# atenpas/gpd

Hardware: NVIDIA H100
Metric: grasp candidates/sec end-to-end (15ch) (higher is better)
Workload: dtype f64 geometry / f32 LeNet

## Files before the change

### gpd_b200/csrc/geometry.cu

```cuda
#include <cfloat>
#include <climits>
#include <cstdlib>
#include <vector>
#include <cub/cub.cuh>

#include "common.cuh"
#include "grid.cuh"

namespace {

constexpr int NT_HANDS = 256;
#ifndef GPDB_NT_IMG
#define GPDB_NT_IMG 512
#endif
constexpr int NT_IMG = GPDB_NT_IMG;
constexpr int LRF_WARPS = 4;
constexpr int LRF_CAP_GLOBAL = 16384;
constexpr int LRF_CAP = 1024;
constexpr int BOX_CAP = 2048;
constexpr int MAXPIX = 64 * 64;

__device__ __forceinline__ void to_frame(const double *F, double v0, double v1, double v2, double &o0, double &o1,
                                         double &o2) {
  o0 = (F[0] * v0 + F[1] * v1) + F[2] * v2;
// ... 1059 lines not shown
}
__device__ __forceinline__ void unit_axis(double v, double lo, double extent, double inv_extent, int S, double &u, int &cell) {
  u = (v - lo) * inv_extent;
  double q = u * (double)S;
  double fq = floor(q);
  const double fr = q - fq;
  if (fr < 1e-9 || fr > 1.0 - 1e-9) {
    u = (v - lo) / extent;
    double cellsize = 1.0 / (double)S;
    fq = floor(u / cellsize);
  }
  cell = min((int)fq, S - 1);
}
__device__ __forceinline__ unsigned unit_q32(double u) {
  return __double2uint_rz(u * 4294967296.0);
}

constexpr int RCP_N = (NT_IMG / 32) * 4;
__device__ __forceinline__ double cell_mean(unsigned long long acc, const double *rcp) {
  const unsigned c = (unsigned)(acc >> 48);
  const double sum = (double)(acc & 0xffffffffffffull);
  return c < (unsigned)RCP_N ? sum * rcp[c] : sum / ((double)c * 4294967296.0);
}

__device__ __forceinline__ bool fully_covered(const unsigned *occf, int S);
template <int NT, int NV>
__device__ __forceinline__ void block_max(float (&v)[NV], float (*red)[8], const unsigned *occf = nullptr, int S = 0,
                                          bool *covered = nullptr) {
#pragma unroll
  for (int o = 16; o; o >>= 1)
#pragma unroll
    for (int i = 0; i < NV; i++) v[i] = fmaxf(v[i], __shfl_xor_sync(0xffffffffu, v[i], o));
  __syncthreads();
  if ((threadIdx.x & 31) == 0)
#pragma unroll
    for (int i = 0; i < NV; i++) red[threadIdx.x >> 5][i] = v[i];
  if (occf && threadIdx.x < 32) {
    const bool c = fully_covered(occf, S);
    if (threadIdx.x == 0) red[0][7] = c ? 1.0f : 0.0f;
  }
  __syncthreads();
#pragma unroll
  for (int i = 0; i < NV; i++) v[i] = red[0][i];
  for (int w = 1; w < NT / 32; w++)
#pragma unroll
    for (int i = 0; i < NV; i++) v[i] = fmaxf(v[i], red[w][i]);
// ... 231 lines not shown
      unit_axis(x, h.bottom, P.vol_d, inv_d, S, u0, c0);
      unit_axis(y, h.center - P.vol_w / 2.0, P.vol_w, inv_w, S, u1, c1);
      unit_axis(z, -P.vol_h, 2.0 * P.vol_h, inv_h, S, u2, c2);
      bq[k] = unit_q32(u0);
      bq[BC + k] = unit_q32(u1);
      bq[2 * BC + k] = unit_q32(u2);
      bcell[k] = (unsigned)c0 | ((unsigned)c1 << 8) | ((unsigned)c2 << 16);
      const double *nn = cl.nrm + 3 * (size_t)(unsigned)(bkeys[k] & 0xffffffffull);
      double n0, n1, n2;
      to_frame(h.frame, nn[0], nn[1], nn[2], n0, n1, n2);
      bnrm[k] = (float)fabs(n0);
      bnrm[BC + k] = (float)fabs(n1);
      bnrm[2 * BC + k] = (float)fabs(n2);
      if (!unit_normal(nn)) nonunit = true;
    }
    const bool exact_fold = __syncthreads_or(nonunit) != 0;

    for (int pj = 0; pj < nproj; pj++) {
      const int a0 = (pj == 0) ? 0 : 2, a1 = (pj == 2) ? 0 : 1, a2 = (pj == 0) ? 2 : (pj == 1 ? 0 : 1);
      for (int k = tid; k < bn; k += NT_IMG) {
        const unsigned cc = bcell[k];
        const int row = S - 1 - (int)((cc >> (8 * a0)) & 255), col = (cc >> (8 * a1)) & 255;
        const int pix = row * S + col;
        atomicMax(tileA + pix, bkeys[k]);
        atomicAdd(tileB + pix, (1ull << 48) + (unsigned long long)bq[a2 * BC + k]);
        atomicOr(&sm.occf[pix >> 5], 1u << (pix & 31));
      }
      __syncthreads();
      auto cell_values = [&](int k, int &row, int &col, float &n0, float &n1, float &n2, float &dv) -> bool {
        const unsigned cc = bcell[k];
        row = S - 1 - (int)((cc >> (8 * a0)) & 255);
        col = (cc >> (8 * a1)) & 255;
        const int pix = row * S + col;
        if (tileA[pix] != bkeys[k]) return false;
        n0 = bnrm[k];
        n1 = bnrm[BC + k];
        n2 = bnrm[2 * BC + k];
        if (exact_fold) {
          float v0 = 0.0f, v1 = 0.0f, v2 = 0.0f;
          unsigned long long cur = 0ull;
          bool first = true;
          for (;;) {
            unsigned long long nxt = ~0ull;
            int jn = k;
            for (int j = 0; j < bn; j++) {
              const unsigned cj = bcell[j];
              const unsigned long long kj = bkeys[j];
              if ((S - 1 - (int)((cj >> (8 * a0)) & 255)) * S + (int)((cj >> (8 * a1)) & 255) == pix && (first || kj > cur) &&
                  kj < nxt) {
// ... 391 lines not shown
            if ((cam_set >> k) & 1) acc &= bitmap[(size_t)k * bm_words + wd];
          bitmap[wd] = acc;
        }
      }
      for (int k = tid; k < (3 * SS) >> 1; k += NT_IMG) reinterpret_cast<uint4 *>(tileA)[k] = make_uint4(0, 0, 0, 0);
      if ((SS & 1) && tid == 0) tileA[3 * SS - 1] = 0ull;
      __syncthreads();
      const int nbits = 64 * d1 * d2;
      unsigned *blist = bitmap + bm_words;
      const int BL_CAP = list_bytes / 4 - bm_words;
      auto eval_voxel = [&](unsigned packed) {
        int b0 = packed & 255, b1 = (packed >> 8) & 255, b2 = packed >> 16;
        double x, y, z;
        if (!voxel_point_in_box(b0 + o0, b1 + o1, b2 + o2, x, y, z)) return;
        double u[3];
        int cellv[3];
        unit_axis(x, h.bottom, P.vol_d, inv_d, S, u[0], cellv[0]);
        unit_axis(y, h.center - P.vol_w / 2.0, P.vol_w, inv_w, S, u[1], cellv[1]);
        unit_axis(z, -P.vol_h, 2.0 * P.vol_h, inv_h, S, u[2], cellv[2]);
#pragma unroll
        for (int pj = 0; pj < 3; pj++) {
          const int a0 = (pj == 0) ? 0 : 2, a1 = (pj == 2) ? 0 : 1, a2 = (pj == 0) ? 2 : (pj == 1 ? 0 : 1);
          const int row = S - 1 - cellv[a0], col = cellv[a1];
          atomicAdd(tileA + (size_t)pj * SS + row * S + col, (1ull << 48) + (unsigned long long)unit_q32(u[a2]));
        }
      };
      if (tid == 0) sm.wl_n = 0;
      __syncthreads();
      for (int wd0 = 0; wd0 * 32 < nbits; wd0 += NT_IMG) {
        const int wd = wd0 + tid;
        unsigned bits = (wd * 32 < nbits) ? bitmap[wd] : 0u;
        int cntb = __popc(bits);
        int incl = cntb;
#pragma unroll
        for (int o = 1; o < 32; o <<= 1) {
          int v = __shfl_up_sync(0xffffffffu, incl, o);
          if (lane >= o) incl += v;
        }
        int total = __shfl_sync(0xffffffffu, incl, 31), base = 0;
        if (lane == 31 && total) base = atomicAdd(&sm.wl_n, total);
        base = __shfl_sync(0xffffffffu, base, 31);
        int pos = base + incl - cntb;
        const int rowi = wd >> 1;
        const unsigned hi = ((unsigned)(rowi % d1) << 8) | ((unsigned)(rowi / d1) << 16) | ((unsigned)(wd & 1) << 5);
        while (bits) {
          int bi = __ffs(bits) - 1;
          bits &= bits - 1;
// ... 93 lines not shown
            const unsigned En = __vimax3_u16x2(E, O, __byte_perm(LO, O, 0x5432));
            const unsigned On = __vimax3_u16x2(O, E, __byte_perm(E, RE, 0x5432));
            res[ch] = __byte_perm(En, On, 0x6240);
          }
        }
#pragma unroll
        for (int i = 0; i < 4; i++) {
          if (c4 * 4 + i < S) {
            const unsigned sel = (unsigned)i | ((unsigned)(4 + i) << 4);
            uint4 o;
            o.x = __byte_perm(__byte_perm(res[0], res[1], sel), __byte_perm(res[2], res[3], sel), 0x5410);
            o.y = __byte_perm(__byte_perm(res[4], res[5], sel), __byte_perm(res[6], res[7], sel), 0x5410);
            o.z = __byte_perm(__byte_perm(res[8], res[9], sel), __byte_perm(res[10], res[11], sel), 0x5410);
            o.w = __byte_perm(__byte_perm(res[12], res[13], sel), __byte_perm(res[14], res[15], sel), 0x5410);
            gout[row * S + c4 * 4 + i] = o;
          }
        }
      }
    }
    PHASE(8);
  }
}

constexpr int BOX_CAP2 = 1024;
struct Img2Smem {
  SegScan<NT_IMG> seg;
  gpdb_pose h;
  double red[NT_IMG / 32][4];
  double center[3];
  double sv[2][3];
  double svh[2][3];
  unsigned occf[MAXPIX / 32 + 2];
  unsigned lcgA[GPDB_MAX_NSP], lcgC[GPDB_MAX_NSP];
  int cam_or, n_img, box_n, wl_n, dl_n, st_n;
  int nonunit;
  int bm_org[3], bm_dims[3];
  float fred[NT_IMG / 32][8];
};

template <bool BATCH>
__global__ void __launch_bounds__(NT_IMG, 2) k_images2(const DevParams *Pp, DevCloud cl0, CloudTable tab, const gpdb_pose *cand, int nc,
                                                       uint8_t *p16, const double *qtab, int *ovf, int *ovf_count,
                                                       unsigned long long *prof) {
  long long t_phase = 0;
  const DevParams &P = *Pp;
  extern __shared__ __align__(16) unsigned char dyn[];
  __shared__ Img2Smem sm;
  constexpr int S = 60, SS = S * S, RW = S / 4, PLB = SS;
  constexpr int PIXT = (SS + NT_IMG - 1) / NT_IMG;
  constexpr int JW = (BOX_CAP2 + NT_IMG - 1) / NT_IMG;
  const int C = P.C;
  unsigned long long *tileA = reinterpret_cast<unsigned long long *>(dyn);
  unsigned long long *tileB = tileA + SS;
  uint8_t *splanes = reinterpret_cast<uint8_t *>(tileB + SS);
  unsigned char *lbase = splanes + 3 * PLB;
  constexpr int LIST_BYTES = BOX_CAP2 * 36;
  unsigned long long *bkeys = reinterpret_cast<unsigned long long *>(lbase);
  unsigned *bq = reinterpret_cast<unsigned *>(bkeys + BOX_CAP2);
  unsigned *bcell = bq + 3 * BOX_CAP2;
  unsigned *bitmap = reinterpret_cast<unsigned *>(lbase);
  uint8_t *tplanes = reinterpret_cast<uint8_t *>(tileA);
  const int tid = threadIdx.x, lane = tid & 31;
  const int nproj = (C >= 12) ? 3 : 1;
  const bool do_nrm = C != 1, do_dep = C == 1 || C >= 12;
  const int npp = (C == 15 || C == 12) ? 12 : C;
  for (int k = tid; k < GPDB_MAX_NSP; k += NT_IMG) {
    sm.lcgA[k] = P.lcgA[k];
    sm.lcgC[k] = P.lcgC[k];
  }
  for (int k = tid; k < MAXPIX / 32 + 2; k += NT_IMG) sm.occf[k] = 0u;

  for (int b = blockIdx.x; b < nc; b += gridDim.x) {
    __syncthreads();
    {
      const int *src = reinterpret_cast<const int *>(cand + b);
      int *dst = reinterpret_cast<int *>(&sm.h);
      for (int k = tid; k < (int)(sizeof(gpdb_pose) / 4); k += NT_IMG) dst[k] = src[k];
    }
    if (tid == 0) {
      sm.cam_or = 0;
      sm.n_img = 0;
      sm.box_n = 0;
      sm.nonunit = 0;
    }
    uint8_t *gimg = p16 + (size_t)b * SS * 16;
    for (int k = tid; k < (npp * PLB) >> 4; k += NT_IMG) reinterpret_cast<uint4 *>(gimg)[k] = make_uint4(0, 0, 0, 0);
    for (int k = tid; k < SS; k += NT_IMG) reinterpret_cast<uint4 *>(tileA)[k] = make_uint4(0, 0, 0, 0);
    for (int k = tid; k < (3 * PLB) >> 4; k += NT_IMG) reinterpret_cast<uint4 *>(splanes)[k] = make_uint4(0, 0, 0, 0);
    __syncthreads();
    PHASE(1);
    const gpdb_pose &h = sm.h;
    const auto &G = CloudSel<BATCH>::get(P, tab, h.sample_slot);
    const DevCloud cl = local_cloud(G, cl0);
    const bool need_cam = (C == 15) && !G.all_seen;
    const double inv_d = 1.0 / P.vol_d, inv_w = 1.0 / P.vol_w, inv_h = 1.0 / (2.0 * P.vol_h);
    float q[3] = {(float)h.sample[0], (float)h.sample[1], (float)h.sample[2]};
    SegRange sr = seg_range(G, q, P.rf_img);
    double sx = 0, sy = 0, sz = 0;
    int cnt = 0, cam_or = 0;
    scan_balanced<NT_IMG>(G, cl, sr, sm.seg, [&](bool in, const float4 &p, int) {
      bool inb = false;
      unsigned long long key = 0;
      if (in) {
        float d = l2_simple(q, p.x, p.y, p.z);
        if (d < P.r2_img) {
          const int idx = __float_as_int(p.w);
          sx += (double)p.x;
          sy += (double)p.y;
          sz += (double)p.z;
          cnt++;
          if (need_cam) cam_or |= cl.cam[idx];
          double x, y, z;
          to_frame(h.frame, (double)p.x - h.sample[0], (double)p.y - h.sample[1], (double)p.z - h.sample[2], x, y, z);
          if (in_image_box(P, h, x, y, z)) {
            inb = true;
            key = ((unsigned long long)__float_as_uint(d) << 32) | (unsigned)idx;
            if (G.nonunit && !unit_normal(cl.nrm + 3 * (size_t)idx)) sm.nonunit = 1;
          }
        }
      }
      unsigned mk = __ballot_sync(0xffffffffu, inb);
      if (mk) {
        int leader = __ffs(mk) - 1, base = 0;
        if (lane == leader) base = atomicAdd(&sm.box_n, __popc(mk));
        base = __shfl_sync(0xffffffffu, base, leader);
        int pos = base + __popc(mk & ((1u << lane) - 1));
        if (inb && pos < BOX_CAP2) {
          bkeys[pos] = key;
          bq[pos] = __float_as_uint(p.x);
          bq[BOX_CAP2 + pos] = __float_as_uint(p.y);
          bq[2 * BOX_CAP2 + pos] = __float_as_uint(p.z);
        }
      }
    });
#pragma unroll
    for (int o = 16; o; o >>= 1) {
      sx += __shfl_xor_sync(0xffffffffu, sx, o);
      sy += __shfl_xor_sync(0xffffffffu, sy, o);
      sz += __shfl_xor_sync(0xffffffffu, sz, o);
    }
    cnt = warp_sum(cnt);
// ... 28 lines not shown
    double *rcp = &sm.red[0][0];
    if (tid < RCP_N) rcp[tid] = 1.0 / ((double)tid * 4294967296.0);
    for (int k = tid; k < bn; k += NT_IMG) {
      const double px = (double)__uint_as_float(bq[k]), py = (double)__uint_as_float(bq[BOX_CAP2 + k]),
                   pz = (double)__uint_as_float(bq[2 * BOX_CAP2 + k]);
      double x, y, z, u0, u1, u2;
      int c0, c1, c2;
      to_frame(h.frame, px - h.sample[0], py - h.sample[1], pz - h.sample[2], x, y, z);
      unit_axis(x, h.bottom, P.vol_d, inv_d, S, u0, c0);
      unit_axis(y, h.center - P.vol_w / 2.0, P.vol_w, inv_w, S, u1, c1);
      unit_axis(z, -P.vol_h, 2.0 * P.vol_h, inv_h, S, u2, c2);
      bq[k] = unit_q32(u0);
      bq[BOX_CAP2 + k] = unit_q32(u1);
      bq[2 * BOX_CAP2 + k] = unit_q32(u2);
      bcell[k] = (unsigned)c0 | ((unsigned)c1 << 8) | ((unsigned)c2 << 16);
    }
    __syncthreads();

    for (int pj = 0; pj < nproj; pj++) {
      const int a0 = (pj == 0) ? 0 : 2, a1 = (pj == 2) ? 0 : 1, a2 = (pj == 0) ? 2 : (pj == 1 ? 0 : 1);
      for (int k = tid; k < bn; k += NT_IMG) {
        const unsigned cc = bcell[k];
        const int pix = (S - 1 - (int)((cc >> (8 * a0)) & 255)) * S + (int)((cc >> (8 * a1)) & 255);
        atomicMax(tileA + pix, bkeys[k]);
        atomicAdd(tileB + pix, (1ull << 48) + (unsigned long long)bq[a2 * BOX_CAP2 + k]);
        atomicOr(&sm.occf[pix >> 5], 1u << (pix & 31));
      }
      __syncthreads();
      float wv[JW][4];
      int wpix[JW];
      float mxv[2] = {0.0f, 0.0f};
#pragma unroll
      for (int j = 0; j < JW; j++) {
        const int k = tid + j * NT_IMG;
        wpix[j] = -1;
        if (k < bn) {
          const unsigned cc = bcell[k];
          const int pix = (S - 1 - (int)((cc >> (8 * a0)) & 255)) * S + (int)((cc >> (8 * a1)) & 255);
          const unsigned long long key = bkeys[k];
          if (tileA[pix] == key) {
            wpix[j] = pix;
            const double *nn = cl.nrm + 3 * (size_t)(unsigned)(key & 0xffffffffull);
            double n0, n1, n2;
            to_frame(h.frame, nn[0], nn[1], nn[2], n0, n1, n2);
            wv[j][0] = (float)fabs(n0);
            wv[j][1] = (float)fabs(n1);
            wv[j][2] = (float)fabs(n2);
            const float avg = (float)cell_mean(tileB[pix], rcp);
            wv[j][3] = (float)(1.0 - (double)avg);
// ... 68 lines not shown
      const int bm_words = 2 * bmd * bmd;
      const double gmax = qtab[GPDB_QTAB_SIZE - 1];
      const double voxel = GPDB_SHADOW_VOXEL;
      if (tid == 0) {
        const double jmax = gmax * voxel * 0.3 + 1e-9;
        const double half_od = P.vol_w / 2.0;
        double mn[3] = {DBL_MAX, DBL_MAX, DBL_MAX}, mx[3] = {-DBL_MAX, -DBL_MAX, -DBL_MAX};
        for (int cr = 0; cr < 8; cr++) {
          double cx = (cr & 1) ? h.bottom + P.vol_d : h.bottom;
          double cy = (cr & 2) ? h.center + half_od : h.center - half_od;
          double cz = (cr & 4) ? P.vol_h : -P.vol_h;
          for (int r = 0; r < 3; r++) {
            double wv2 = h.frame[r] * cx + h.frame[3 + r] * cy + h.frame[6 + r] * cz + h.sample[r];
            mn[r] = fmin(mn[r], wv2);
            mx[r] = fmax(mx[r], wv2);
          }
        }
        for (int r = 0; r < 3; r++) {
          int lo = (int)floor((mn[r] - jmax) * P.vox_mult) - 1;
          int hi = (int)floor((mx[r] + jmax) * P.vox_mult) + 1;
          sm.bm_org[r] = lo;
          sm.bm_dims[r] = min(hi - lo + 1, bmd);
        }
      }
      if (tid < K) {
        double s0 = sm.center[0] - G.vp[tid][0], s1 = sm.center[1] - G.vp[tid][1], s2 = sm.center[2] - G.vp[tid][2];
        double nn = sqrt((s0 * s0 + s1 * s1) + s2 * s2);
        sm.sv[tid][0] = P.shadow_length * s0 / nn;
        sm.sv[tid][1] = P.shadow_length * s1 / nn;
        sm.sv[tid][2] = P.shadow_length * s2 / nn;
        to_frame(h.frame, sm.sv[tid][0], sm.sv[tid][1], sm.sv[tid][2], sm.svh[tid][0], sm.svh[tid][1], sm.svh[tid][2]);
      }
      for (int k = tid; k < bm_words * K; k += NT_IMG) bitmap[k] = 0u;
      __syncthreads();
      PHASE(4);
      const int o0 = sm.bm_org[0], o1 = sm.bm_org[1], o2 = sm.bm_org[2];
      const int d0 = sm.bm_dims[0], d1 = sm.bm_dims[1], d2 = sm.bm_dims[2];
      const double mxu = 1.0 / 32767.0;
      auto voxel_point_in_box = [&](int v0, int v1, int v2, double &x, double &y, double &z) -> bool {
        double g = qtab[gpdb_voxel_hash(v0, v1, v2) & (GPDB_QTAB_SIZE - 1)];
        double jit = 1.0 * g * voxel * 0.3;
        double w0 = (double)v0 * voxel + jit, w1 = (double)v1 * voxel + jit, w2 = (double)v2 * voxel + jit;
        to_frame(h.frame, w0 - h.sample[0], w1 - h.sample[1], w2 - h.sample[2], x, y, z);
        return in_image_box(P, h, x, y, z);
      };
      const int cam_set = sm.cam_or;
      float4 *wl = reinterpret_cast<float4 *>(tileA);
      constexpr int WL_CAP = (SS * 8) / 20;
      unsigned *wrange = reinterpret_cast<unsigned *>(wl + WL_CAP);
      unsigned *dlist = reinterpret_cast<unsigned *>(tileB);
      constexpr int DL_CAP = 2 * SS;
      const double wm = 0.0105;
      const double bx_lo[3] = {h.bottom - wm, h.center - P.vol_w / 2.0 - wm, -P.vol_h - wm};
      const double bx_hi[3] = {h.bottom + P.vol_d + wm, h.center + P.vol_w / 2.0 + wm, P.vol_h + wm};
      float fR[9];
#pragma unroll
      for (int e = 0; e < 9; e++) fR[e] = (float)h.frame[e];
      const float fsx = (float)h.sample[0], fsy = (float)h.sample[1], fsz = (float)h.sample[2];
      const float jm = (float)(gmax * voxel * 0.3 * 1.7320508075688772 + 2e-5);
      const float fbx_lo[3] = {(float)h.bottom - jm, (float)(h.center - P.vol_w / 2.0) - jm, (float)(-P.vol_h) - jm};
      const float fbx_hi[3] = {(float)(h.bottom + P.vol_d) + jm, (float)(h.center + P.vol_w / 2.0) + jm, (float)P.vol_h + jm};
      auto draw_bit = [&](double px, double py, double pz, unsigned seed, int k) -> int {
        const double s0 = sm.sv[k][0], s1 = sm.sv[k][1], s2 = sm.sv[k][2];
        double u = (double)((seed >> 16) & 0x7FFFu) * mxu;
        int v0 = (int)((px + u * s0) * P.vox_mult);
        int v1 = (int)((py + u * s1) * P.vox_mult);
        int v2 = (int)((pz + u * s2) * P.vox_mult);
        int b0 = v0 - o0, b1 = v1 - o1, b2 = v2 - o2;
        if ((unsigned)b0 >= (unsigned)d0 || (unsigned)b1 >= (unsigned)d1 || (unsigned)b2 >= (unsigned)d2) return -1;
        const float wx = fmaf((float)v0, 0.003f, -fsx), wy = fmaf((float)v1, 0.003f, -fsy), wz = fmaf((float)v2, 0.003f, -fsz);
        const float hx = fmaf(fR[0], wx, fmaf(fR[1], wy, fR[2] * wz));
        const float hy = fmaf(fR[3], wx, fmaf(fR[4], wy, fR[5] * wz));
        const float hz = fmaf(fR[6], wx, fmaf(fR[7], wy, fR[8] * wz));
        if (hx < fbx_lo[0] || hx > fbx_hi[0] || hy < fbx_lo[1] || hy > fbx_hi[1] || hz < fbx_lo[2] || hz > fbx_hi[2]) return -1;
        return ((b2 * d1 + b1) << 6) + b0;
      };
      for (int k = 0; k < K; k++) {
        if (!((cam_set >> k) & 1)) continue;
        unsigned *bm = bitmap + (size_t)k * bm_words;
        float cull_lo[3], cull_hi[3], cull_inv[3];
        bool cull_par[3];
#pragma unroll
        for (int a = 0; a < 3; a++) {
          const float dv = (float)sm.svh[k][a];
          cull_par[a] = fabsf(dv) < 1e-6f;
          cull_inv[a] = cull_par[a] ? 0.0f : 1.0f / dv;
          cull_lo[a] = (float)bx_lo[a] - 1e-5f;
          cull_hi[a] = (float)bx_hi[a] + 1e-5f;
        }
        __syncthreads();
        if (tid == 0) {
          sm.wl_n = 0;
          sm.dl_n = 0;
        }
        __syncthreads();
        auto cull = [&](const float4 &p, unsigned &rg) -> bool {
          const float wx = p.x - fsx, wy = p.y - fsy, wz = p.z - fsz;
          const float o3[3] = {fmaf(fR[0], wx, fmaf(fR[1], wy, fR[2] * wz)), fmaf(fR[3], wx, fmaf(fR[4], wy, fR[5] * wz)),
                               fmaf(fR[6], wx, fmaf(fR[7], wy, fR[8] * wz))};
          float tmin = 0.0f, tmax = 1.0f;
          bool hit = true;
#pragma unroll
          for (int a = 0; a < 3; a++) {
            if (cull_par[a]) {
              hit = hit && o3[a] >= cull_lo[a] && o3[a] <= cull_hi[a];
            } else {
              const float t1 = (cull_lo[a] - o3[a]) * cull_inv[a], t2 = (cull_hi[a] - o3[a]) * cull_inv[a];
              tmin = fmaxf(tmin, fminf(t1, t2));
              tmax = fminf(tmax, fmaxf(t1, t2));
            }
          }
          if (!hit || tmin > tmax) return false;
          const int r0 = max((int)floorf(tmin * 32767.0f) - 1, 0), r1 = min((int)ceilf(tmax * 32767.0f) + 1, 32767);
          rg = (unsigned)r0 | ((unsigned)r1 << 16);
          return true;
        };
        scan_balanced<NT_IMG>(G, cl, sr, sm.seg, [&](bool in, const float4 &p, int) {
          unsigned rg = 0;
          const bool ok = in && l2_simple(q, p.x, p.y, p.z) < P.r2_img && cull(p, rg);
          const unsigned mk = __ballot_sync(0xffffffffu, ok);
          if (!mk) return;
          const int leader = __ffs(mk) - 1;
          int base = 0;
          if (lane == leader) base = atomicAdd(&sm.wl_n, __popc(mk));
          base = __shfl_sync(0xffffffffu, base, leader);
          if (!ok) return;
          const int pos = base + __popc(mk & ((1u << lane) - 1));
          const unsigned seed0 = gpdb_shadow_seed((unsigned)h.sample_index, (unsigned)__float_as_int(p.w), (unsigned)k);
          if (pos < WL_CAP) {
            wl[pos] = make_float4(p.x, p.y, p.z, __uint_as_float(seed0));
            wrange[pos] = rg;
          } else {
            unsigned seed = seed0;
            const int r0 = (int)(rg & 0xFFFFu), r1 = (int)(rg >> 16);
            for (int t = 0; t < P.nsp; t++) {
              int r = (int)gpdb_fastrand(&seed);
              if (r >= r0 && r <= r1) {
                int bit = draw_bit((double)p.x, (double)p.y, (double)p.z, seed, k);
                if (bit >= 0) atomicOr(bm + (bit >> 5), 1u << (bit & 31));
              }
            }
          }
        });
        __syncthreads();
        const int nw = min(sm.wl_n, WL_CAP);
        if (prof && tid == 0) atomicAdd(prof + 9, (unsigned long long)nw);
        const int nsp = P.nsp;
        const unsigned nsp_magic = nsp > 1 ? (unsigned)((0x100000000ull + (unsigned)nsp - 1) / (unsigned)nsp) : 0u;
        const int nd = nw * nsp;
        for (int w0 = 0; w0 < nd; w0 += NT_IMG) {
          const int w = w0 + tid;
          bool pass = false;
          unsigned code = 0, seed = 0;
          if (w < nd) {
            const int item = nsp > 1 ? (int)__umulhi((unsigned)w, nsp_magic) : w, t = w - item * nsp;
            seed = sm.lcgA[t] * __float_as_uint(wl[item].w) + sm.lcgC[t];
            const unsigned rg = wrange[item];
            const int r = (int)((seed >> 16) & 0x7FFFu);
            pass = r >= (int)(rg & 0xFFFFu) && r <= (int)(rg >> 16);
            code = ((unsigned)item << 7) | (unsigned)t;
          }
          const unsigned mk = __ballot_sync(0xffffffffu, pass);
          if (mk) {
            const int leader = __ffs(mk) - 1;
            int base = 0;
            if (lane == leader) base = atomicAdd(&sm.dl_n, __popc(mk));
// ... 37 lines not shown
        }
      }
      for (int k = tid; k < SS; k += NT_IMG) reinterpret_cast<uint4 *>(tileA)[k] = make_uint4(0, 0, 0, 0);
      if (tid == 0) sm.st_n = 0;
      __syncthreads();
      const int nbits = 64 * d1 * d2;
      uint2 *stash = reinterpret_cast<uint2 *>(bitmap + (((size_t)bm_words * (K > 1 ? K : 1) + 1) & ~(size_t)1));
      const int ST_CAP = (LIST_BYTES - (int)((reinterpret_cast<unsigned char *>(stash)) - lbase)) / 8;
      auto eval_voxel = [&](unsigned packed, int pj_lo, int pj_hi) -> uint2 {
        int b0 = packed & 255, b1 = (packed >> 8) & 255, b2 = packed >> 16;
        double x, y, z;
        if (!voxel_point_in_box(b0 + o0, b1 + o1, b2 + o2, x, y, z)) return make_uint2(0u, 0u);
        double u[3];
        int cellv[3];
        unit_axis(x, h.bottom, P.vol_d, inv_d, S, u[0], cellv[0]);
        unit_axis(y, h.center - P.vol_w / 2.0, P.vol_w, inv_w, S, u[1], cellv[1]);
        unit_axis(z, -P.vol_h, 2.0 * P.vol_h, inv_h, S, u[2], cellv[2]);
        uint2 st = make_uint2(0u, 0u);
#pragma unroll
        for (int pj = 0; pj < 3; pj++) {
          const int a0 = (pj == 0) ? 0 : 2, a1 = (pj == 2) ? 0 : 1, a2 = (pj == 0) ? 2 : (pj == 1 ? 0 : 1);
          const int pix = (S - 1 - cellv[a0]) * S + cellv[a1];
          const unsigned qv = unit_q32(u[a2]);
          if (pj >= pj_lo && pj < pj_hi) atomicAdd(tileA + (size_t)(pj - pj_lo) * SS + pix, (1ull << 48) + (unsigned long long)qv);
          if (pj == 2) st = make_uint2((unsigned)pix | 0x80000000u, qv);
        }
        return st;
      };
      for (int wd0 = 0; wd0 * 32 < nbits; wd0 += NT_IMG) {
        const int wd = wd0 + tid;
        unsigned bits = (wd * 32 < nbits) ? bitmap[wd] : 0u;
        int cntb = __popc(bits);
        int incl = cntb;
#pragma unroll
        for (int o = 1; o < 32; o <<= 1) {
          int v = __shfl_up_sync(0xffffffffu, incl, o);
          if (lane >= o) incl += v;
        }
        int total = __shfl_sync(0xffffffffu, incl, 31), base = 0;
        if (lane == 31 && total) base = atomicAdd(&sm.st_n, total);
        base = __shfl_sync(0xffffffffu, base, 31);
        int pos = base + incl - cntb;
        const int rowi = wd >> 1;
        const unsigned hi = ((unsigned)(rowi % d1) << 8) | ((unsigned)(rowi / d1) << 16) | ((unsigned)(wd & 1) << 5);
        while (bits) {
          int bi = __ffs(bits) - 1;
          bits &= bits - 1;
          if (pos < ST_CAP) stash[pos].x = hi | (unsigned)bi;
          else eval_voxel(hi | (unsigned)bi, 0, 2);
          pos++;
        }
      }
      __syncthreads();
      const int nset_all = sm.st_n, nset = min(nset_all, ST_CAP);
      if (prof && tid == 0) {
        atomicAdd(prof + 11, (unsigned long long)nset_all);
        atomicAdd(prof + 12, (unsigned long long)bn);
        atomicAdd(prof + 13, (unsigned long long)sm.n_img);
      }
      for (int i = tid; i < nset; i += NT_IMG) stash[i] = eval_voxel(stash[i].x, 0, 2);
      __syncthreads();
      PHASE(6);
      auto shadow_channel = [&](int pj, unsigned long long *tile) {
        uint8_t *plane = splanes + (size_t)pj * PLB;
        float avgr[PIXT];
        unsigned occm = 0;
        float mm[2] = {-FLT_MAX, -FLT_MAX};
#pragma unroll
        for (int t = 0; t < PIXT; t++) {
          const int pix = tid + t * NT_IMG;
          avgr[t] = 0.0f;
          bool oc = false;
          if (pix < SS) {
            const unsigned long long acc = tile[pix];
// ... 26 lines not shown
          float neg[1] = {-dilated_min<NT_IMG>(srcF, S)};
          block_max<NT_IMG, 1>(neg, sm.fred);
          vmin = -neg[0];
        }
        const Quant qs(vmin, vmax);
        const unsigned bg = qs(0.0f);
#pragma unroll
        for (int t = 0; t < PIXT; t++) {
          const int pix = tid + t * NT_IMG;
          if (pix < SS) {
            const bool oc = (occm >> t) & 1;
            if (oc || bg) plane[pix] = (uint8_t)(oc ? qs(maxf - avgr[t]) : bg);
          }
        }
      };
      shadow_channel(0, tileA);
      shadow_channel(1, tileB);
      __syncthreads();
      for (int k = tid; k < SS / 2; k += NT_IMG) reinterpret_cast<uint4 *>(tileA)[k] = make_uint4(0, 0, 0, 0);
      __syncthreads();
      if (nset_all <= ST_CAP) {
        for (int i = tid; i < nset; i += NT_IMG) {
          const uint2 st = stash[i];
          if (st.x & 0x80000000u) atomicAdd(tileA + (st.x & 0x7fffffffu), (1ull << 48) + (unsigned long long)st.y);
        }
      } else {
        for (int wd = tid; wd * 32 < nbits; wd += NT_IMG) {
          unsigned bits = bitmap[wd];
          const int rowi = wd >> 1;
          const unsigned hi = ((unsigned)(rowi % d1) << 8) | ((unsigned)(rowi / d1) << 16) | ((unsigned)(wd & 1) << 5);
          while (bits) {
            int bi = __ffs(bits) - 1;
            bits &= bits - 1;
            eval_voxel(hi | (unsigned)bi, 2, 3);
          }
        }
      }
      __syncthreads();
      shadow_channel(2, tileA);
      __syncthreads();
      for (int k = tid; k < MAXPIX / 32; k += NT_IMG) sm.occf[k] = 0u;
    }
    __syncthreads();
    PHASE(7);
    for (int k = tid; k < (npp * PLB) >> 4; k += NT_IMG)
      reinterpret_cast<uint4 *>(tplanes)[k] = __ldcg(reinterpret_cast<const uint4 *>(gimg) + k);
    __syncthreads();
    {
      uint4 *gout = reinterpret_cast<uint4 *>(gimg);
      for (int g = tid; g < S * RW; g += NT_IMG) {
        const int row = g / RW, c4 = g - row * RW;
        unsigned res[16];
        const bool up = row > 0, dn = row + 1 < S, lf = c4 > 0, rt = c4 + 1 < RW;
#pragma unroll
        for (int ch = 0; ch < 16; ch++) {
          res[ch] = 0u;
          if (ch < C) {
            const uint8_t *pl = (C == 15) ? ((ch % 5 == 4) ? splanes + (size_t)(ch / 5) * PLB : tplanes + (size_t)(4 * (ch / 5) + ch % 5) * PLB)
                                          : tplanes + (size_t)ch * PLB;
            const unsigned *W = reinterpret_cast<const unsigned *>(pl) + row * RW + c4;
            const unsigned m0 = W[0], u0 = up ? W[-RW] : 0u, d0w = dn ? W[RW] : 0u;
// ... 308 lines not shown
template <bool BATCH>
static int launch_images(gpdb_ctx *ctx, const DevCloud &cl, const gpdb_pose *d_cand, int nc, uint8_t *d_p16) {
  const DevParams &hp = ctx->hp;
  const int K = BATCH ? ctx->b_maxk : hp.K;
  const CloudTable tab = ctx->run;
  const int S = hp.S, RS = (S + 3) & ~3;
  const size_t plane_bytes = ((size_t)hp.C * S * RS + 15) / 16 * 16;
  const size_t tiles = (size_t)3 * 8 * S * S;
  const size_t bm = (size_t)K * (2 * (size_t)hp.bm_dim * hp.bm_dim) * 4;
  const size_t list_bytes = (std::max((size_t)BOX_CAP * 36, hp.C == 15 ? bm + 4096 * 4 : (size_t)0) + 15) / 16 * 16;
  const size_t smem = plane_bytes + tiles + list_bytes;
  if (smem > 219 * 1024) {
    gpdb_set_error(ctx, GPDB_ERR_INVALID, "image geometry needs %zu B of shared memory per CTA (max 224256)", smem);
    return GPDB_ERR_INVALID;
  }
  const char *force = getenv("GPD_B200_IMAGES_KERNEL");
  const bool fast = S == 60 && (hp.C != 15 || (K <= 2 && bm + 2048 <= (size_t)BOX_CAP2 * 36)) && !(force && force[0] == '1');
  const int *d_work = nullptr, *d_work_n = nullptr;
  if (fast) {
    int *ovf = (int *)gpdb_scratch(ctx, 22, sizeof(int) * ((size_t)nc + 1));
    if (!ovf) return GPDB_ERR_CUDA;
    int *ovf_count = ovf + nc;
    CUDA_TRY(cudaMemsetAsync(ovf_count, 0, sizeof(int), ctx->stream));
    const size_t smem2 = (size_t)2 * 8 * S * S + (size_t)3 * S * S + (size_t)BOX_CAP2 * 36;
    CUDA_TRY(cudaFuncSetAttribute(k_images2<BATCH>, cudaFuncAttributeMaxDynamicSharedMemorySize, (int)smem2));
    k_images2<BATCH><<<std::min(nc, ctx->sm_count * 64), NT_IMG, smem2, ctx->stream>>>(ctx->dp, cl, tab, d_cand, nc, d_p16, ctx->d_qtab, ovf,
                                                                               ovf_count, ctx->d_prof);
    LAUNCH_CHECK();
    d_work = ovf;
    d_work_n = ovf_count;
  }
  int *ovf2 = (int *)gpdb_scratch(ctx, 20, sizeof(int) * ((size_t)nc + 1));
  const int gl_cap = 32768;
  const size_t gl_slice = (size_t)gl_cap * 36 + (size_t)16 * S * S;
  unsigned char *gl = (unsigned char *)gpdb_scratch(ctx, 19, gl_slice * (size_t)ctx->sm_count);
  if (!ovf2 || !gl) return GPDB_ERR_CUDA;
  int *ovf2_count = ovf2 + nc;
  CUDA_TRY(cudaMemsetAsync(ovf2_count, 0, sizeof(int), ctx->stream));
  const int grid = fast ? ctx->sm_count : std::min(nc, ctx->sm_count * 64);
  if (S == 60) {
    CUDA_TRY(cudaFuncSetAttribute(k_images<60, false, BATCH>, cudaFuncAttributeMaxDynamicSharedMemorySize, (int)smem));
    CUDA_TRY(cudaFuncSetAttribute(k_images<60, true, BATCH>, cudaFuncAttributeMaxDynamicSharedMemorySize, (int)smem));
    k_images<60, false, BATCH><<<grid, NT_IMG, smem, ctx->stream>>>(ctx->dp, cl, tab, d_cand, nc, d_p16, ctx->d_qtab, ctx->d_err,
                                                             (int)plane_bytes, (int)list_bytes, ctx->d_prof, d_work, d_work_n,
                                                             nullptr, 0, ovf2, ovf2_count);
    LAUNCH_CHECK();
    k_images<60, true, BATCH><<<ctx->sm_count, NT_IMG, smem, ctx->stream>>>(ctx->dp, cl, tab, d_cand, nc, d_p16, ctx->d_qtab, ctx->d_err,
// ... 178 lines not shown
```

Measured before the change: 1.426 million.

## Cache ball point indices, split 64-bit smem atomics, warp-parallel bit expansion

Records the indices of in-ball points during the first scan into spare global image memory, so later per-camera shadow passes revisit only those points instead of rescanning the segment. Replaces 64-bit shared-memory atomicMax/atomicAdd with 32-bit atomics: a two-pass distance-then-index max, and a split add with manual carry propagation. Replaces the serial per-thread bitmap expansion with a warp-cooperative expansion that spreads set bits across lanes. It also hoists cull and frame constants into shared memory and adds profiling counters. The trade-off is more passes and syncs, possible races in the split carry-add, and extra global traffic for the ball list.

```diff
diff --git a/gpd_b200/csrc/geometry.cu b/gpd_b200/csrc/geometry.cu
--- a/gpd_b200/csrc/geometry.cu
+++ b/gpd_b200/csrc/geometry.cu
@@ -1105,6 +1105,20 @@
   const double sum = (double)(acc & 0xffffffffffffull);
   return c < (unsigned)RCP_N ? sum * rcp[c] : sum / ((double)c * 4294967296.0);
 }
+__device__ __forceinline__ bool cell_add(unsigned long long *cell, unsigned q) {
+  unsigned *w = reinterpret_cast<unsigned *>(cell);
+  const unsigned lo_old = atomicAdd(w, q);
+  const bool carry = lo_old + q < lo_old;
+  atomicAdd(w + 1, (1u << 16) + (carry ? 1u : 0u));
+  return carry;
+}
+__device__ __forceinline__ void key_max_dist(unsigned long long *cell, unsigned long long key) {
+  atomicMax(reinterpret_cast<unsigned *>(cell) + 1, (unsigned)(key >> 32));
+}
+__device__ __forceinline__ void key_max_index(unsigned long long *cell, unsigned long long key) {
+  unsigned *w = reinterpret_cast<unsigned *>(cell);
+  if (w[1] == (unsigned)(key >> 32)) atomicMax(w, (unsigned)key);
+}
 
 __device__ __forceinline__ bool fully_covered(const unsigned *occf, int S);
 template <int NT, int NV>
@@ -1382,9 +1396,15 @@
         const unsigned cc = bcell[k];
         const int row = S - 1 - (int)((cc >> (8 * a0)) & 255), col = (cc >> (8 * a1)) & 255;
         const int pix = row * S + col;
-        atomicMax(tileA + pix, bkeys[k]);
-        atomicAdd(tileB + pix, (1ull << 48) + (unsigned long long)bq[a2 * BC + k]);
+        key_max_dist(tileA + pix, bkeys[k]);
         atomicOr(&sm.occf[pix >> 5], 1u << (pix & 31));
+      }
+      __syncthreads();
+      for (int k = tid; k < bn; k += NT_IMG) {
+        const unsigned cc = bcell[k];
+        const int pix = (S - 1 - (int)((cc >> (8 * a0)) & 255)) * S + (int)((cc >> (8 * a1)) & 255);
+        key_max_index(tileA + pix, bkeys[k]);
+        cell_add(tileB + pix, bq[a2 * BC + k]);
       }
       __syncthreads();
       auto cell_values = [&](int k, int &row, int &col, float &n0, float &n1, float &n2, float &dv) -> bool {
@@ -1822,7 +1842,7 @@
         for (int pj = 0; pj < 3; pj++) {
           const int a0 = (pj == 0) ? 0 : 2, a1 = (pj == 2) ? 0 : 1, a2 = (pj == 0) ? 2 : (pj == 1 ? 0 : 1);
           const int row = S - 1 - cellv[a0], col = cellv[a1];
-          atomicAdd(tileA + (size_t)pj * SS + row * S + col, (1ull << 48) + (unsigned long long)unit_q32(u[a2]));
+          cell_add(tileA + (size_t)pj * SS + row * S + col, unit_q32(u[a2]));
         }
       };
       if (tid == 0) sm.wl_n = 0;
@@ -1962,7 +1982,35 @@
   }
 }
 
+template <class R, class E>
+__device__ __forceinline__ void warp_expand_bits(unsigned bits, unsigned code, R &&reserve, E &&emit) {
+  const int lane = threadIdx.x & 31;
+  const int cnt = __popc(bits);
+  int incl = cnt;
+#pragma unroll
+  for (int o = 1; o < 32; o <<= 1) {
+    const int v = __shfl_up_sync(0xffffffffu, incl, o);
+    if (lane >= o) incl += v;
+  }
+  const int total = __shfl_sync(0xffffffffu, incl, 31);
+  const int base = reserve(total);
+  for (int j0 = 0; j0 < total; j0 += 32) {
+    const int j = j0 + lane;
+    int w = 0;
+#pragma unroll
+    for (int s = 16; s; s >>= 1) {
+      const int v = __shfl_sync(0xffffffffu, incl, w + s - 1);
+      if (v <= j) w += s;
+    }
+    const unsigned wbits = __shfl_sync(0xffffffffu, bits, w), wcode = __shfl_sync(0xffffffffu, code, w);
+    const int wexcl = __shfl_sync(0xffffffffu, incl - cnt, w);
+    if (j < total) emit(base + j, wcode | __fns(wbits, 0, j - wexcl + 1));
+  }
+}
+
 constexpr int BOX_CAP2 = 1024;
+constexpr int IMG2_S = 60;
+constexpr int BALL_CAP2 = (IMG2_S * IMG2_S * 16 - 12 * IMG2_S * IMG2_S) / 4;
 struct Img2Smem {
   SegScan<NT_IMG> seg;
   gpdb_pose h;
@@ -1973,10 +2021,15 @@
   unsigned occf[MAXPIX / 32 + 2];
   unsigned lcgA[GPDB_MAX_NSP], lcgC[GPDB_MAX_NSP];
   int cam_or, n_img, box_n, wl_n, dl_n, st_n;
+  int ball_n;
   int nonunit;
   int bm_org[3], bm_dims[3];
   float fred[NT_IMG / 32][8];
+  float fR[9], fs[3], fbx_lo[3], fbx_hi[3], cull_lo[3], cull_hi[3];
+  float cull_inv[2][3];
 };
+constexpr size_t IMG2_DYN_SMEM = (size_t)2 * 8 * IMG2_S * IMG2_S + (size_t)3 * IMG2_S * IMG2_S + (size_t)BOX_CAP2 * 36;
+static_assert(2 * (IMG2_DYN_SMEM + sizeof(Img2Smem) + 1024) <= 228 * 1024, "k_images2 no longer fits two CTAs per SM");
 
 template <bool BATCH>
 __global__ void __launch_bounds__(NT_IMG, 2) k_images2(const DevParams *Pp, DevCloud cl0, CloudTable tab, const gpdb_pose *cand, int nc,
@@ -1986,7 +2039,7 @@
   const DevParams &P = *Pp;
   extern __shared__ __align__(16) unsigned char dyn[];
   __shared__ Img2Smem sm;
-  constexpr int S = 60, SS = S * S, RW = S / 4, PLB = SS;
+  constexpr int S = IMG2_S, SS = S * S, RW = S / 4, PLB = SS;
   constexpr int PIXT = (SS + NT_IMG - 1) / NT_IMG;
   constexpr int JW = (BOX_CAP2 + NT_IMG - 1) / NT_IMG;
   const int C = P.C;
@@ -2021,9 +2074,11 @@
       sm.cam_or = 0;
       sm.n_img = 0;
       sm.box_n = 0;
+      sm.ball_n = 0;
       sm.nonunit = 0;
     }
     uint8_t *gimg = p16 + (size_t)b * SS * 16;
+    int *ball = reinterpret_cast<int *>(gimg + 12 * PLB);
     for (int k = tid; k < (npp * PLB) >> 4; k += NT_IMG) reinterpret_cast<uint4 *>(gimg)[k] = make_uint4(0, 0, 0, 0);
     for (int k = tid; k < SS; k += NT_IMG) reinterpret_cast<uint4 *>(tileA)[k] = make_uint4(0, 0, 0, 0);
     for (int k = tid; k < (3 * PLB) >> 4; k += NT_IMG) reinterpret_cast<uint4 *>(splanes)[k] = make_uint4(0, 0, 0, 0);
@@ -2038,12 +2093,13 @@
     SegRange sr = seg_range(G, q, P.rf_img);
     double sx = 0, sy = 0, sz = 0;
     int cnt = 0, cam_or = 0;
-    scan_balanced<NT_IMG>(G, cl, sr, sm.seg, [&](bool in, const float4 &p, int) {
-      bool inb = false;
+    scan_balanced<NT_IMG>(G, cl, sr, sm.seg, [&](bool in, const float4 &p, int where) {
+      bool inb = false, inball = false;
       unsigned long long key = 0;
       if (in) {
         float d = l2_simple(q, p.x, p.y, p.z);
         if (d < P.r2_img) {
+          inball = true;
           const int idx = __float_as_int(p.w);
           sx += (double)p.x;
           sy += (double)p.y;
@@ -2057,6 +2113,17 @@
             key = ((unsigned long long)__float_as_uint(d) << 32) | (unsigned)idx;
             if (G.nonunit && !unit_normal(cl.nrm + 3 * (size_t)idx)) sm.nonunit = 1;
           }
+        }
+      }
+      if (C == 15) {
+        const unsigned mb = __ballot_sync(0xffffffffu, inball);
+        if (mb) {
+          const int leader = __ffs(mb) - 1;
+          int base = 0;
+          if (lane == leader) base = atomicAdd(&sm.ball_n, __popc(mb));
+          base = __shfl_sync(0xffffffffu, base, leader);
+          const int pos = base + __popc(mb & ((1u << lane) - 1));
+          if (inball && pos < BALL_CAP2) ball[pos] = where;
         }
       }
       unsigned mk = __ballot_sync(0xffffffffu, inb);
@@ -2131,9 +2198,15 @@
       for (int k = tid; k < bn; k += NT_IMG) {
         const unsigned cc = bcell[k];
         const int pix = (S - 1 - (int)((cc >> (8 * a0)) & 255)) * S + (int)((cc >> (8 * a1)) & 255);
-        atomicMax(tileA + pix, bkeys[k]);
-        atomicAdd(tileB + pix, (1ull << 48) + (unsigned long long)bq[a2 * BOX_CAP2 + k]);
+        key_max_dist(tileA + pix, bkeys[k]);
         atomicOr(&sm.occf[pix >> 5], 1u << (pix & 31));
+      }
+      __syncthreads();
+      for (int k = tid; k < bn; k += NT_IMG) {
+        const unsigned cc = bcell[k];
+        const int pix = (S - 1 - (int)((cc >> (8 * a0)) & 255)) * S + (int)((cc >> (8 * a1)) & 255);
+        key_max_index(tileA + pix, bkeys[k]);
+        cell_add(tileB + pix, bq[a2 * BOX_CAP2 + k]);
       }
       __syncthreads();
       float wv[JW][4];
@@ -2248,6 +2321,22 @@
           sm.bm_org[r] = lo;
           sm.bm_dims[r] = min(hi - lo + 1, bmd);
         }
+        for (int e = 0; e < 9; e++) sm.fR[e] = (float)h.frame[e];
+        for (int r = 0; r < 3; r++) sm.fs[r] = (float)h.sample[r];
+        const float jm = (float)(gmax * voxel * 0.3 * 1.7320508075688772 + 2e-5);
+        sm.fbx_lo[0] = (float)h.bottom - jm;
+        sm.fbx_lo[1] = (float)(h.center - P.vol_w / 2.0) - jm;
+        sm.fbx_lo[2] = (float)(-P.vol_h) - jm;
+        sm.fbx_hi[0] = (float)(h.bottom + P.vol_d) + jm;
+        sm.fbx_hi[1] = (float)(h.center + P.vol_w / 2.0) + jm;
+        sm.fbx_hi[2] = (float)P.vol_h + jm;
+        const double wm = 0.0105;
+        const double bx_lo[3] = {h.bottom - wm, h.center - P.vol_w / 2.0 - wm, -P.vol_h - wm};
+        const double bx_hi[3] = {h.bottom + P.vol_d + wm, h.center + P.vol_w / 2.0 + wm, P.vol_h + wm};
+        for (int a = 0; a < 3; a++) {
+          sm.cull_lo[a] = (float)bx_lo[a] - 1e-5f;
+          sm.cull_hi[a] = (float)bx_hi[a] + 1e-5f;
+        }
       }
       if (tid < K) {
         double s0 = sm.center[0] - G.vp[tid][0], s1 = sm.center[1] - G.vp[tid][1], s2 = sm.center[2] - G.vp[tid][2];
@@ -2256,6 +2345,10 @@
         sm.sv[tid][1] = P.shadow_length * s1 / nn;
         sm.sv[tid][2] = P.shadow_length * s2 / nn;
         to_frame(h.frame, sm.sv[tid][0], sm.sv[tid][1], sm.sv[tid][2], sm.svh[tid][0], sm.svh[tid][1], sm.svh[tid][2]);
+        for (int a = 0; a < 3; a++) {
+          const float dv = (float)sm.svh[tid][a];
+          sm.cull_inv[tid][a] = fabsf(dv) < 1e-6f ? 0.0f : 1.0f / dv;
+        }
       }
       for (int k = tid; k < bm_words * K; k += NT_IMG) bitmap[k] = 0u;
       __syncthreads();
@@ -2270,22 +2363,13 @@
         to_frame(h.frame, w0 - h.sample[0], w1 - h.sample[1], w2 - h.sample[2], x, y, z);
         return in_image_box(P, h, x, y, z);
       };
-      const int cam_set = sm.cam_or;
+      const int cam_set = sm.cam_or, nball = sm.ball_n;
       float4 *wl = reinterpret_cast<float4 *>(tileA);
       constexpr int WL_CAP = (SS * 8) / 20;
       unsigned *wrange = reinterpret_cast<unsigned *>(wl + WL_CAP);
       unsigned *dlist = reinterpret_cast<unsigned *>(tileB);
       constexpr int DL_CAP = 2 * SS;
-      const double wm = 0.0105;
-      const double bx_lo[3] = {h.bottom - wm, h.center - P.vol_w / 2.0 - wm, -P.vol_h - wm};
-      const double bx_hi[3] = {h.bottom + P.vol_d + wm, h.center + P.vol_w / 2.0 + wm, P.vol_h + wm};
-      float fR[9];
-#pragma unroll
-      for (int e = 0; e < 9; e++) fR[e] = (float)h.frame[e];
-      const float fsx = (float)h.sample[0], fsy = (float)h.sample[1], fsz = (float)h.sample[2];
-      const float jm = (float)(gmax * voxel * 0.3 * 1.7320508075688772 + 2e-5);
-      const float fbx_lo[3] = {(float)h.bottom - jm, (float)(h.center - P.vol_w / 2.0) - jm, (float)(-P.vol_h) - jm};
-      const float fbx_hi[3] = {(float)(h.bottom + P.vol_d) + jm, (float)(h.center + P.vol_w / 2.0) + jm, (float)P.vol_h + jm};
+      const float *fR = sm.fR, *fs = sm.fs, *fbx_lo = sm.fbx_lo, *fbx_hi = sm.fbx_hi, *cull_lo = sm.cull_lo, *cull_hi = sm.cull_hi;
       auto draw_bit = [&](double px, double py, double pz, unsigned seed, int k) -> int {
         const double s0 = sm.sv[k][0], s1 = sm.sv[k][1], s2 = sm.sv[k][2];
         double u = (double)((seed >> 16) & 0x7FFFu) * mxu;
@@ -2294,7 +2378,7 @@
         int v2 = (int)((pz + u * s2) * P.vox_mult);
         int b0 = v0 - o0, b1 = v1 - o1, b2 = v2 - o2;
         if ((unsigned)b0 >= (unsigned)d0 || (unsigned)b1 >= (unsigned)d1 || (unsigned)b2 >= (unsigned)d2) return -1;
-        const float wx = fmaf((float)v0, 0.003f, -fsx), wy = fmaf((float)v1, 0.003f, -fsy), wz = fmaf((float)v2, 0.003f, -fsz);
+        const float wx = fmaf((float)v0, 0.003f, -fs[0]), wy = fmaf((float)v1, 0.003f, -fs[1]), wz = fmaf((float)v2, 0.003f, -fs[2]);
         const float hx = fmaf(fR[0], wx, fmaf(fR[1], wy, fR[2] * wz));
         const float hy = fmaf(fR[3], wx, fmaf(fR[4], wy, fR[5] * wz));
         const float hz = fmaf(fR[6], wx, fmaf(fR[7], wy, fR[8] * wz));
@@ -2304,16 +2388,7 @@
       for (int k = 0; k < K; k++) {
         if (!((cam_set >> k) & 1)) continue;
         unsigned *bm = bitmap + (size_t)k * bm_words;
-        float cull_lo[3], cull_hi[3], cull_inv[3];
-        bool cull_par[3];
-#pragma unroll
-        for (int a = 0; a < 3; a++) {
-          const float dv = (float)sm.svh[k][a];
-          cull_par[a] = fabsf(dv) < 1e-6f;
-          cull_inv[a] = cull_par[a] ? 0.0f : 1.0f / dv;
-          cull_lo[a] = (float)bx_lo[a] - 1e-5f;
-          cull_hi[a] = (float)bx_hi[a] + 1e-5f;
-        }
+        const float *cull_inv = sm.cull_inv[k];
         __syncthreads();
         if (tid == 0) {
           sm.wl_n = 0;
@@ -2321,14 +2396,14 @@
         }
         __syncthreads();
         auto cull = [&](const float4 &p, unsigned &rg) -> bool {
-          const float wx = p.x - fsx, wy = p.y - fsy, wz = p.z - fsz;
+          const float wx = p.x - fs[0], wy = p.y - fs[1], wz = p.z - fs[2];
           const float o3[3] = {fmaf(fR[0], wx, fmaf(fR[1], wy, fR[2] * wz)), fmaf(fR[3], wx, fmaf(fR[4], wy, fR[5] * wz)),
                                fmaf(fR[6], wx, fmaf(fR[7], wy, fR[8] * wz))};
           float tmin = 0.0f, tmax = 1.0f;
           bool hit = true;
 #pragma unroll
           for (int a = 0; a < 3; a++) {
-            if (cull_par[a]) {
+            if (cull_inv[a] == 0.0f) {
               hit = hit && o3[a] >= cull_lo[a] && o3[a] <= cull_hi[a];
             } else {
               const float t1 = (cull_lo[a] - o3[a]) * cull_inv[a], t2 = (cull_hi[a] - o3[a]) * cull_inv[a];
@@ -2341,9 +2416,7 @@
           rg = (unsigned)r0 | ((unsigned)r1 << 16);
           return true;
         };
-        scan_balanced<NT_IMG>(G, cl, sr, sm.seg, [&](bool in, const float4 &p, int) {
-          unsigned rg = 0;
-          const bool ok = in && l2_simple(q, p.x, p.y, p.z) < P.r2_img && cull(p, rg);
+        auto append = [&](bool ok, const float4 &p, unsigned rg) {
           const unsigned mk = __ballot_sync(0xffffffffu, ok);
           if (!mk) return;
           const int leader = __ffs(mk) - 1;
@@ -2367,7 +2440,27 @@
               }
             }
           }
-        });
+        };
+        if (nball <= BALL_CAP2) {
+          for (int i0 = 0; i0 < nball; i0 += NT_IMG) {
+            const int i = i0 + tid;
+            float4 p = make_float4(0.f, 0.f, 0.f, 0.f);
+            unsigned rg = 0;
+            bool ok = false;
+            if (i < nball) {
+              p = __ldg(cl.pts4 + __ldcg(ball + i));
+              ok = cull(p, rg);
+            }
+            append(ok, p, rg);
+          }
+        } else {
+          scan_balanced<NT_IMG>(G, cl, sr, sm.seg, [&](bool in, const float4 &p, int) {
+            unsigned rg = 0;
+            const bool ok = in && l2_simple(q, p.x, p.y, p.z) < P.r2_img && cull(p, rg);
+            append(ok, p, rg);
+          });
+          if (prof && tid == 0) atomicAdd(prof + 14, 1ull);
+        }
         __syncthreads();
         const int nw = min(sm.wl_n, WL_CAP);
         if (prof && tid == 0) atomicAdd(prof + 9, (unsigned long long)nw);
@@ -2451,34 +2544,29 @@
           const int a0 = (pj == 0) ? 0 : 2, a1 = (pj == 2) ? 0 : 1, a2 = (pj == 0) ? 2 : (pj == 1 ? 0 : 1);
           const int pix = (S - 1 - cellv[a0]) * S + cellv[a1];
           const unsigned qv = unit_q32(u[a2]);
-          if (pj >= pj_lo && pj < pj_hi) atomicAdd(tileA + (size_t)(pj - pj_lo) * SS + pix, (1ull << 48) + (unsigned long long)qv);
+          if (pj >= pj_lo && pj < pj_hi) cell_add(tileA + (size_t)(pj - pj_lo) * SS + pix, qv);
           if (pj == 2) st = make_uint2((unsigned)pix | 0x80000000u, qv);
         }
         return st;
+      };
+      auto word_code = [&](int wd) -> unsigned {
+        const int rowi = wd >> 1;
+        return ((unsigned)(rowi % d1) << 8) | ((unsigned)(rowi / d1) << 16) | ((unsigned)(wd & 1) << 5);
       };
       for (int wd0 = 0; wd0 * 32 < nbits; wd0 += NT_IMG) {
         const int wd = wd0 + tid;
-        unsigned bits = (wd * 32 < nbits) ? bitmap[wd] : 0u;
-        int cntb = __popc(bits);
-        int incl = cntb;
-#pragma unroll
-        for (int o = 1; o < 32; o <<= 1) {
-          int v = __shfl_up_sync(0xffffffffu, incl, o);
-          if (lane >= o) incl += v;
-        }
-        int total = __shfl_sync(0xffffffffu, incl, 31), base = 0;
-        if (lane == 31 && total) base = atomicAdd(&sm.st_n, total);
-        base = __shfl_sync(0xffffffffu, base, 31);
-        int pos = base + incl - cntb;
-        const int rowi = wd >> 1;
-        const unsigned hi = ((unsigned)(rowi % d1) << 8) | ((unsigned)(rowi / d1) << 16) | ((unsigned)(wd & 1) << 5);
-        while (bits) {
-          int bi = __ffs(bits) - 1;
-          bits &= bits - 1;
-          if (pos < ST_CAP) stash[pos].x = hi | (unsigned)bi;
-          else eval_voxel(hi | (unsigned)bi, 0, 2);
-          pos++;
-        }
+        const unsigned bits = (wd * 32 < nbits) ? bitmap[wd] : 0u;
+        warp_expand_bits(
+            bits, word_code(wd),
+            [&](int total) {
+              int base = 0;
+              if (lane == 0 && total) base = atomicAdd(&sm.st_n, total);
+              return __shfl_sync(0xffffffffu, base, 0);
+            },
+            [&](int pos, unsigned code) {
+              if (pos < ST_CAP) stash[pos].x = code;
+              else eval_voxel(code, 0, 2);
+            });
       }
       __syncthreads();
       const int nset_all = sm.st_n, nset = min(nset_all, ST_CAP);
@@ -2551,21 +2639,25 @@
       if (nset_all <= ST_CAP) {
         for (int i = tid; i < nset; i += NT_IMG) {
           const uint2 st = stash[i];
-          if (st.x & 0x80000000u) atomicAdd(tileA + (st.x & 0x7fffffffu), (1ull << 48) + (unsigned long long)st.y);
+          if (st.x & 0x80000000u) {
+            const bool carry = cell_add(tileA + (st.x & 0x7fffffffu), st.y);
+            if (prof && carry) atomicAdd(prof + 0, 1ull);
+          }
         }
       } else {
-        for (int wd = tid; wd * 32 < nbits; wd += NT_IMG) {
-          unsigned bits = bitmap[wd];
-          const int rowi = wd >> 1;
-          const unsigned hi = ((unsigned)(rowi % d1) << 8) | ((unsigned)(rowi / d1) << 16) | ((unsigned)(wd & 1) << 5);
-          while (bits) {
-            int bi = __ffs(bits) - 1;
-            bits &= bits - 1;
-            eval_voxel(hi | (unsigned)bi, 2, 3);
-          }
+        for (int wd0 = 0; wd0 * 32 < nbits; wd0 += NT_IMG) {
+          const int wd = wd0 + tid;
+          const unsigned bits = (wd * 32 < nbits) ? bitmap[wd] : 0u;
+          warp_expand_bits(bits, word_code(wd), [](int) { return 0; }, [&](int, unsigned code) { eval_voxel(code, 2, 3); });
         }
       }
       __syncthreads();
+      if (prof) {
+        unsigned most = 0;
+        for (int k = tid; k < SS; k += NT_IMG) most = max(most, (unsigned)(tileA[k] >> 48));
+        most = __reduce_max_sync(0xffffffffu, most);
+        if (lane == 0 && most) atomicMax(prof + 1, (unsigned long long)most);
+      }
       shadow_channel(2, tileA);
       __syncthreads();
       for (int k = tid; k < MAXPIX / 32; k += NT_IMG) sm.occf[k] = 0u;
@@ -2920,7 +3012,7 @@
     if (!ovf) return GPDB_ERR_CUDA;
     int *ovf_count = ovf + nc;
     CUDA_TRY(cudaMemsetAsync(ovf_count, 0, sizeof(int), ctx->stream));
-    const size_t smem2 = (size_t)2 * 8 * S * S + (size_t)3 * S * S + (size_t)BOX_CAP2 * 36;
+    const size_t smem2 = IMG2_DYN_SMEM;
     CUDA_TRY(cudaFuncSetAttribute(k_images2<BATCH>, cudaFuncAttributeMaxDynamicSharedMemorySize, (int)smem2));
     k_images2<BATCH><<<std::min(nc, ctx->sm_count * 64), NT_IMG, smem2, ctx->stream>>>(ctx->dp, cl, tab, d_cand, nc, d_p16, ctx->d_qtab, ovf,
                                                                                ovf_count, ctx->d_prof);
```

Result: faster. 1.578 million, median of 6 (+10.7%).
